# wheretrue/exon

Hardware: AMD Instinct MI355X
Metric: Mrows/sec filter+agg on 1B-row synthetic VCF; achieved HBM GB/s vs peak (higher is better)
Workload: dtype f64

## Files before the change

### exon_amd/_lib.py

```python
import ctypes as C
import os
import subprocess

_HERE = os.path.dirname(os.path.abspath(__file__))
LIB_PATH = os.environ.get("EXON_HIP_LIB") or os.path.join(_HERE, "lib", "libexon_hip.so")
CSRC = os.path.join(_HERE, "csrc")


class ExonHipError(RuntimeError):
    def __init__(self, code, msg):
        super().__init__(f"exon_hip status {code}: {msg}")
        self.code = code


class ArrowSchema(C.Structure):
    pass


ArrowSchema._fields_ = [
    ("format", C.c_char_p), ("name", C.c_char_p), ("metadata", C.c_char_p), ("flags", C.c_int64),
    ("n_children", C.c_int64), ("children", C.POINTER(C.POINTER(ArrowSchema))),
    ("dictionary", C.POINTER(ArrowSchema)), ("release", C.c_void_p), ("private_data", C.c_void_p),
]

# ... 39 lines not shown
        ("lmax", C.c_int32), ("y_type", C.c_int32),
        ("columns", C.c_int32 * 4),
    ]


class BgzfBlock(C.Structure):
    _fields_ = [("comp_offset", C.c_uint32), ("comp_size", C.c_uint32), ("out_offset", C.c_uint32), ("out_size", C.c_uint32),
                ("crc32", C.c_uint32), ("reserved", C.c_uint32)]


class BAMColumns(C.Structure):
    _fields_ = [("n_rows", C.c_int64), ("n_undecided", C.c_int64), ("consumed_bytes", C.c_int64), ("flag", C.c_void_p),
                ("mapq", C.c_void_p), ("mapq_valid", C.c_void_p), ("ref_id", C.c_void_p), ("ref_valid", C.c_void_p),
                ("start", C.c_void_p), ("end", C.c_void_p), ("pos_valid", C.c_void_p)]


class FASTQViews(C.Structure):
    _fields_ = [("n_reads", C.c_int64), ("n_undecided", C.c_int64), ("consumed_bytes", C.c_int64),
                ("seq_start", C.c_void_p), ("seq_end", C.c_void_p), ("qual_start", C.c_void_p), ("qual_end", C.c_void_p),
                ("text_base", C.c_void_p), ("head_start", C.c_void_p), ("head_end", C.c_void_p)]


class FASTAViews(C.Structure):
    _fields_ = [("n_records", C.c_int64), ("n_undecided", C.c_int64), ("consumed_bytes", C.c_int64), ("n_lines", C.c_int64),
                ("seq_bytes", C.c_int64), ("text_base", C.c_void_p), ("text_bytes", C.c_int64), ("first_line_start", C.c_int64),
                ("head_start", C.c_void_p), ("head_end", C.c_void_p), ("seq_offsets", C.c_void_p), ("line_end", C.c_void_p),
                ("line_dst", C.c_void_p)]


class VCFColumns(C.Structure):
    _fields_ = [("n_rows", C.c_int64), ("n_undecided", C.c_int64), ("chrom_id", C.c_void_p), ("pos", C.c_void_p),
                ("pos_valid", C.c_void_p), ("qual", C.c_void_p), ("qual_valid", C.c_void_p), ("filter_id", C.c_void_p),
                ("info", C.c_void_p), ("info_valid", C.c_void_p), ("consumed_bytes", C.c_int64),
                ("n_info", C.c_int32), ("reserved", C.c_int32), ("infos", C.c_void_p * 16), ("infos_valid", C.c_void_p * 16),
                ("info_kinds", C.c_char * 16), ("list_offsets", C.c_void_p * 16), ("list_item_valid", C.c_void_p * 16),
                ("info_nulls", C.c_int32 * 16)]


class GFFColumns(C.Structure):
    _fields_ = [("n_rows", C.c_int64), ("n_undecided", C.c_int64), ("consumed_bytes", C.c_int64),
                ("seqname_id", C.c_void_p), ("source_id", C.c_void_p), ("type_id", C.c_void_p), ("start", C.c_void_p),
                ("end", C.c_void_p), ("score", C.c_void_p), ("score_valid", C.c_void_p), ("strand_id", C.c_void_p),
                ("strand_valid", C.c_void_p), ("phase_id", C.c_void_p), ("phase_valid", C.c_void_p)]


class GFFAttributes(C.Structure):
    _fields_ = [("n_entries", C.c_int64), ("n_items", C.c_int64), ("n_key_bytes", C.c_int64), ("n_item_bytes", C.c_int64),
                ("n_undecided", C.c_int64), ("map_offsets", C.c_void_p), ("key_offsets", C.c_void_p), ("key_values", C.c_void_p),
                ("list_offsets", C.c_void_p), ("item_offsets", C.c_void_p), ("item_values", C.c_void_p)]


class VCFInfoText(C.Structure):
    _fields_ = [("n_bytes", C.c_int64), ("n_undecided", C.c_int64), ("offsets", C.c_void_p), ("values", C.c_void_p)]


class GTFAttributes(C.Structure):
    _fields_ = [("n_entries", C.c_int64), ("n_key_bytes", C.c_int64), ("n_value_bytes", C.c_int64), ("n_undecided", C.c_int64),
                ("map_offsets", C.c_void_p), ("key_offsets", C.c_void_p), ("key_values", C.c_void_p),
                ("value_offsets", C.c_void_p), ("value_values", C.c_void_p)]


class BEDColumns(C.Structure):
    _fields_ = [("n_rows", C.c_int64), ("n_undecided", C.c_int64), ("consumed_bytes", C.c_int64),
                ("chrom_id", C.c_void_p), ("start", C.c_void_p), ("end", C.c_void_p), ("score", C.c_void_p), ("score_valid", C.c_void_p),
                ("strand_id", C.c_void_p), ("strand_valid", C.c_void_p), ("name_off", C.c_void_p), ("name_len", C.c_void_p),
                ("name_valid", C.c_void_p), ("text", C.c_void_p)]


class ScanOptions(C.Structure):
    _fields_ = [("format", C.c_int32), ("compression", C.c_int32), ("batch_size", C.c_int64),
                ("info_field", C.c_char_p), ("region", C.c_char_p), ("use_index", C.c_int32), ("gpu_parse", C.c_int32),
                ("projection", C.c_uint64)]


class GzipStats(C.Structure):
    _fields_ = [(n, C.c_uint64) for n in ("calls", "chunks", "repairs", "overflow_retries", "members", "comp_bytes", "out_bytes")]


FORMATS = {"vcf": 1, "bam": 2, "fastq": 3, "fasta": 4, "sam": 5, "bcf": 6, "cram": 7, "gff": 8, "gtf": 9, "bed": 10}
COMPRESSION = {"auto": 0, None: 0, "none": 1, "gzip": 2}
PROJECT_VCF_FORMATS_ON_DEVICE = 32
PROJECT_BED = {"name": 1 << 3, "score": 1 << 4, "strand": 1 << 5, "thick_start": 1 << 6, "thick_end": 1 << 7, "color": 1 << 8,
               "block_count": 1 << 9, "block_sizes": 1 << 10, "block_starts": 1 << 11}

PLAN_REGION_COUNT = 2
PLAN_FLAG_MAPQ_GROUP_COUNT = 3
PLAN_CMP_AVG_BY_GROUP = 4
PLAN_QUAL_POS_HIST = 5
PLAN_OVERLAP_COUNT = 6
PLAN_WITHIN_COUNT = 7
PLAN_CMP_MINMAX_BY_GROUP = 8
PLAN_READ_STATS_HIST = 9
PLAN_SEQ_STATS_HIST = 10
LAUNCH_ACCUMULATE = 0
LAUNCH_OVERWRITE = 1
CMP = {">": 0, ">=": 1, "<": 2, "<=": 3, "=": 4, "==": 4, "!=": 5, "<>": 5}
REGION_OPEN_END = 2**63 - 1

_vp, _i32, _i64, _u64, _dbl = C.c_void_p, C.c_int32, C.c_int64, C.c_uint64, C.c_double
_colp = C.POINTER(Column)

ALLGATHER_FN = C.CFUNCTYPE(C.c_int, C.c_void_p, C.c_void_p, C.c_void_p, C.c_size_t)

SIGNATURES = {
    "exon_hip_abi_version": (C.c_int, []),
    "exon_hip_device_count": (C.c_int, [C.POINTER(C.c_int)]),
    "exon_hip_ctx_create": (C.c_int, [C.c_int, C.POINTER(_vp)]),
    "exon_hip_ctx_destroy": (C.c_int, [_vp]),
    "exon_hip_ctx_info": (C.c_int, [_vp, C.POINTER(DeviceInfo)]),
    "exon_hip_last_error": (C.c_char_p, [_vp]),
    "exon_hip_malloc": (C.c_int, [_vp, C.c_size_t, C.POINTER(_vp)]),
    "exon_hip_free": (C.c_int, [_vp, _vp]),
    "exon_hip_memcpy_h2d": (C.c_int, [_vp, _vp, _vp, C.c_size_t, _vp]),
    "exon_hip_memcpy_d2h": (C.c_int, [_vp, _vp, _vp, C.c_size_t, _vp]),
    "exon_hip_memset": (C.c_int, [_vp, _vp, C.c_int, C.c_size_t, _vp]),
    "exon_hip_sync": (C.c_int, [_vp, _vp]),
    "exon_hip_read_probe": (C.c_int, [_vp, _vp, C.POINTER(_vp), _i32, _i64, _i32, C.POINTER(_dbl), C.POINTER(_i64)]),
    "exon_hip_timer_start": (C.c_int, [_vp, _vp]),
    "exon_hip_timer_stop_ms": (C.c_int, [_vp, _vp, C.POINTER(C.c_float)]),
    "exon_hip_region_count": (C.c_int, [_vp, _vp, _colp, _colp, _i64, _i32, _i64, _i64, _vp]),
    "exon_hip_overlap_count": (C.c_int, [_vp, _vp, _colp, _colp, _colp, _i64, _i32, _i64, _i64, _vp]),
    "exon_hip_within_count": (C.c_int, [_vp, _vp, _colp, _colp, _colp, _i64, _i32, _i64, _i64, _vp]),
    "exon_hip_flag_mapq_group_count": (C.c_int, [_vp, _vp, _colp, _colp, _colp, _i64, _i32, _i32, _i32, _i32, _vp]),
    "exon_hip_cmp_avg_by_group": (C.c_int, [_vp, _vp, _colp, _colp, _colp, _i64, _dbl, _i32, _i32, _vp, _vp]),
    "exon_hip_cmp_minmax_by_group": (C.c_int, [_vp, _vp, _colp, _colp, _colp, _i64, _dbl, _i32, _i32, _vp]),
    "exon_hip_minmax_decode": (C.c_int, [_vp, _i64, _i32, _i32, _vp, _vp]),
    "exon_hip_qual_pos_hist": (C.c_int, [_vp, _vp, _colp, _i64, _i32, _vp]),
    "exon_hip_gen_c6": (C.c_int, [_vp, _vp, _u64, _i64, _i64, _vp, _vp, _vp, _vp, _vp]),
    "exon_hip_gen_c2": (C.c_int, [_vp, _vp, _u64, _i64, _i64, _i64, _vp, _vp]),
    "exon_hip_gen_c3": (C.c_int, [_vp, _vp, _u64, _i64, _i64, _vp, _vp, _vp, _vp, _vp]),
    "exon_hip_gen_c4": (C.c_int, [_vp, _vp, _u64, _i64, _i64, _vp, _vp, _vp, _vp, _vp]),
    "exon_hip_gen_c5": (C.c_int, [_vp, _vp, _u64, _i64, _i64, _i32, _vp, _vp]),
    "exon_hip_parse_region": (C.c_int, [C.c_char_p, C.c_char_p, C.c_size_t, C.POINTER(_i64), C.POINTER(_i64)]),
    "exon_hip_regroup_files_by_size": (C.c_int, [C.POINTER(_i64), _i32, _i32, C.POINTER(_i32)]),
    "exon_hip_plan_create": (C.c_int, [_vp, C.POINTER(PlanDesc), C.POINTER(_vp)]),
    "exon_hip_plan_destroy": (C.c_int, [_vp]),
    "exon_hip_plan_state_size": (C.c_int, [_vp, C.POINTER(_i64), C.POINTER(_i64)]),
    "exon_hip_plan_launch": (C.c_int, [_vp, _vp, _colp, _i32, _i64, _i32, _vp]),
    "exon_hip_plan_launch_chunks": (C.c_int, [_vp, _vp, _colp, _i32, _i32, _vp, _i32, _vp]),
    "exon_hip_fold_states": (C.c_int, [_vp, _vp, _vp, _i32, _i64, _i64, _vp]),
    "exon_hip_merge_states": (C.c_int, [_vp, _vp, _vp, _vp, _i64, _i64, _vp, _vp]),
    "exon_hip_plan_fold_states": (C.c_int, [_vp, _vp, _vp, _i32, _vp]),
    "exon_hip_rccl_unique_id": (C.c_int, [_vp]),
    "exon_hip_rccl_comm_init": (C.c_int, [_vp, _vp, _i32, _i32, C.POINTER(_vp)]),
    "exon_hip_rccl_comm_destroy": (C.c_int, [_vp]),
    "exon_hip_comm_wrap_rccl": (C.c_int, [_vp, C.POINTER(_vp)]),
    "exon_hip_comm_from_callbacks": (C.c_int, [_i32, _i32, ALLGATHER_FN, _vp, C.POINTER(_vp)]),
    "exon_hip_rccl_comm_count": (C.c_int, [_vp, C.POINTER(_i32), C.POINTER(_i32)]),
    "exon_hip_stream_reset": (C.c_int, [_vp]),
    "exon_hip_stream_open": (C.c_int, [_vp, _i32, C.POINTER(_vp)]),
    "exon_hip_stream_push": (C.c_int, [_vp, C.POINTER(ArrowArray)]),
    "exon_hip_stream_push_device": (C.c_int, [_vp, C.POINTER(ArrowDeviceArray)]),
    "exon_hip_stream_state": (C.c_int, [_vp, C.POINTER(_vp), C.POINTER(_vp), C.POINTER(_vp)]),
    "exon_hip_stream_all_reduce": (C.c_int, [_vp, _vp]),
    "exon_hip_stream_keys": (C.c_int, [_vp, _vp, C.c_size_t, C.POINTER(_i32), C.POINTER(C.c_size_t), C.POINTER(_i32)]),
    "exon_hip_stream_set_keys": (C.c_int, [_vp, C.c_char_p, C.c_size_t, _i32]),
    "exon_hip_keys_union": (C.c_int, [C.c_char_p, C.c_size_t, C.POINTER(_i32), _i32, _vp, C.c_size_t, C.POINTER(_i32),
                                      C.POINTER(C.c_size_t), C.POINTER(_i32)]),
    "exon_hip_stream_reconcile_keys": (C.c_int, [_vp, _vp]),
    "exon_hip_stream_set_region_contig": (C.c_int, [_vp, C.c_char_p]),
    "exon_hip_stream_sync": (C.c_int, [_vp]),
    "exon_hip_stream_finish": (C.c_int, [_vp, _vp, _vp]),
    "exon_hip_stream_finish_arrow": (C.c_int, [_vp, C.POINTER(ArrowArray), C.POINTER(ArrowSchema)]),
    "exon_hip_stream_close": (C.c_int, [_vp]),
    "exon_hip_scan_open": (C.c_int, [C.c_char_p, C.POINTER(ScanOptions), C.POINTER(_vp)]),
    "exon_hip_scan_schema": (C.c_int, [_vp, C.POINTER(ArrowSchema)]),
# ... 101 lines not shown
```

### exon_amd/csrc/gpu_parse.hip

```cpp
#include <hip/hip_runtime.h>

#include <cstring>
#include <string>
#include <vector>

#include "host/decimal_f32.h"
#include "internal.h"
#include "list_kernels.h"

namespace {

constexpr int TPB = 256;
constexpr int FILTER_SLOTS = 8192;
constexpr int FILTER_POOL = EXON_DICT_POOL;

__host__ __device__ inline uint64_t fnv1a(const uint8_t* p, int n) {
  uint64_t h = 0xCBF29CE484222325ULL;
  for (int i = 0; i < n; ++i) {
    h ^= p[i];
    h *= 0x100000001B3ULL;
  }
  return h | 1ULL;
}

// ... 175 lines not shown
  }
  int read_back(exon_hip_ctx* ctx, hipStream_t s) {
    HIP_TRY(ctx, hipGetLastError());
    HIP_TRY(ctx, hipMemcpyAsync(h_scalars, d_scalars, 16, hipMemcpyDeviceToHost, s));
    HIP_TRY(ctx, hipStreamSynchronize(s));
    return EXON_HIP_OK;
  }
  int64_t consumed(unsigned skip) const { return h_scalars[2] > skip ? (int64_t)h_scalars[2] - skip : 0; }
};

__global__ void k_last_newline(const unsigned* __restrict__ nl_pos, unsigned* __restrict__ scalars, unsigned cap) {
  const unsigned n = scalars[0];
  scalars[2] = (n && n <= cap) ? nl_pos[n - 1] + 1u : 0u;
}

struct NameTable {
  const uint64_t* keys;
  const int32_t* ids;
  const uint32_t* text_off;
  const uint32_t* text_len;
  const uint8_t* pool;
  int mask;
};

struct FilterTable {
  unsigned long long* keys;
  int32_t* ids;
  uint32_t* text_off;
  uint32_t* text_len;
  uint8_t* pool;
  int32_t* counters;
};

constexpr int MAX_INFO = EXON_HIP_MAX_INFO_FIELDS;
struct InfoKeys {
  int n;
  int len[MAX_INFO];
  int off[MAX_INFO];
  char kind[MAX_INFO];
  const uint8_t* text;
};
struct ParseOut {
  int32_t* chrom_id;
  int64_t* pos;
  uint8_t* pos_valid;
  float* qual;
  uint8_t* qual_valid;
  int32_t* filter_id;
  uint32_t* filter_off;
  uint32_t* filter_len;
  float* info[MAX_INFO];
  uint8_t* info_valid[MAX_INFO];
  uint32_t* lv_off[MAX_INFO];
  uint32_t* lv_cnt[MAX_INFO];
  unsigned* exceptions;
};

__device__ __forceinline__ void store_valid(uint8_t* bm, int64_t row0_of_wave, int64_t n_rows, bool v, int lane) {
  const unsigned long long m = __ballot(v);
  if (lane < 8) {
    const int64_t r = row0_of_wave + lane * 8;
    if (r < n_rows) bm[r >> 3] = (uint8_t)(m >> (lane * 8));
  }
}

__device__ __forceinline__ unsigned eq_mask16(const uint4& v, uint32_t splat) {
  const uint32_t w[4] = {v.x, v.y, v.z, v.w};
  unsigned mask = 0;
#pragma unroll
  for (int k = 0; k < 4; ++k) {
    const uint32_t x = w[k] ^ splat;
    const uint32_t m = ~(((x & 0x7F7F7F7Fu) + 0x7F7F7F7Fu) | x | 0x7F7F7F7Fu);
    const uint32_t t = m >> 7;
    mask |= ((t | (t >> 7) | (t >> 14) | (t >> 21)) & 0xFu) << (4 * k);
  }
  return mask;
}
__device__ __forceinline__ unsigned clip_mask16(unsigned mask, unsigned a, unsigned begin, unsigned end) {
  if (begin > a) mask &= 0xFFFFu << (begin - a);
  if (end - a < 16u) mask &= (1u << (end - a)) - 1u;
  return mask;
}

__global__ __launch_bounds__(TPB) void k_parse_lines(const uint8_t* __restrict__ text, const unsigned* __restrict__ nl_pos,
                                                     const unsigned* __restrict__ n_lines_p, NameTable contigs,
                                                     FilterTable filters, InfoKeys ik, ParseOut out, unsigned cap, unsigned skip,
                                                     unsigned n_total) {
  const int64_t n_rows = min(*n_lines_p, cap);
  auto group16 = [&](unsigned a) {
    uint4 v = {0, 0, 0, 0};
    if (a + 16u <= n_total) {
      v = *reinterpret_cast<const uint4*>(text + a);
    } else {
      unsigned* w = &v.x;
      for (unsigned i = 0; a + i < n_total; ++i) w[i >> 2] |= (unsigned)text[a + i] << (8 * (i & 3));
    }
    return v;
  };
  const int64_t row = (int64_t)blockIdx.x * TPB + threadIdx.x;
  const int lane = threadIdx.x & 63;
  bool pos_ok = false, qual_ok = false, bad = false;
  unsigned info_ok = 0;
  if (row < n_rows) {
    const unsigned begin = row ? nl_pos[row - 1] + 1 : skip;
    unsigned end = nl_pos[row];
    if (end > begin && text[end - 1] == '\r') --end;
    unsigned fs[9];
    int nf = 0;
    fs[0] = begin;
    for (unsigned a = begin & ~15u; a < end && nf < 8; a += 16) {
      unsigned m = clip_mask16(eq_mask16(group16(a), 0x09090909u), a, begin, end);
      while (m && nf < 8) {
        fs[++nf] = a + (unsigned)__ffs((int)m);
        m &= m - 1;
      }
    }
    auto fbeg = [&](int f) { return fs[f]; };
    auto fend = [&](int f) { return f < nf ? fs[f + 1] - 1 : end; };
    if (nf < 7 || begin == end || text[begin] == '#') {
      bad = true;
      out.chrom_id[row] = 0;
      out.pos[row] = 0;
      out.qual[row] = 0.f;
      out.filter_id[row] = -1;
      for (int q = 0; q < ik.n; ++q)
        if (ik.kind[q] == 'F' || ik.kind[q] == 'I') out.lv_cnt[q][row] = 0;
    } else {
#ifndef EXON_PARSE_SKIP
#define EXON_PARSE_SKIP 0
#endif
      if (!(EXON_PARSE_SKIP & 1)) {
        const uint8_t* p = text + fbeg(0);
        const int len = (int)(fend(0) - fbeg(0));
        const uint64_t h = fnv1a(p, len);
        int slot = (int)(h & (uint64_t)contigs.mask), id = -1;
        for (int probe = 0; probe <= contigs.mask; ++probe) {
          const uint64_t k = contigs.keys[slot];
          if (k == 0) break;
          if (k == h && (int)contigs.text_len[slot] == len) {
            bool same = true;
            for (int i = 0; i < len && same; ++i) same = contigs.pool[contigs.text_off[slot] + i] == p[i];
            if (same) {
              id = contigs.ids[slot];
              break;
            }
          }
          slot = (slot + 1) & contigs.mask;
        }
        if (id < 0) bad = true;
        out.chrom_id[row] = id < 0 ? 0 : id;
      }
      if (!(EXON_PARSE_SKIP & 2)) {
        uint64_t v = 0;
        unsigned pb = fbeg(1), pn = fend(1) - fbeg(1);
        if (pn && text[pb] == '+') ++pb, --pn;
        bool ok = pn > 0;
        if (pn <= 16 && pb + 16u <= n_total) {
          uint64_t w[2];
          __builtin_memcpy(w, text + pb, 16);
          for (unsigned k = 0; k < pn; ++k) {
            const unsigned d = ((unsigned)(w[k >> 3] >> (8 * (k & 7))) & 0xFFu) - (unsigned)'0';
            ok &= d <= 9u;
            v = v * 10 + d;
          }
        } else {
          for (unsigned i = pb; i < pb + pn && ok; ++i) {
            const uint8_t c = text[i];
            if (c < '0' || c > '9') ok = false;
            else v = v * 10 + (c - '0');
          }
        }
        if (pn > 18) ok = false;
        pos_ok = ok && v > 0;
        if (!ok) bad = true;
        out.pos[row] = pos_ok ? (int64_t)v : 0;
      }
      if (!(EXON_PARSE_SKIP & 4)) {
        const int len = (int)(fend(5) - fbeg(5));
        float q = 0.f;
        if (!(len == 1 && text[fbeg(5)] == '.')) {
          uint32_t bits;
          if (exon::dec::parse_f32(reinterpret_cast<const char*>(text + fbeg(5)), len, &bits)) {
            q = __uint_as_float(bits);
            qual_ok = true;
          } else {
            bad = true;
          }
        }
        out.qual[row] = q;
      }
      if (!(EXON_PARSE_SKIP & 8)) {
        const uint8_t* p = text + fbeg(6);
        int len = (int)(fend(6) - fbeg(6));
        if (len == 1 && p[0] == '.') len = 0;
        const unsigned long long h = fnv1a(p, len);
        int slot = (int)(h & (FILTER_SLOTS - 1));
        int found = -1;
        for (int probe = 0; probe < FILTER_SLOTS; ++probe) {
          unsigned long long k = filters.keys[slot];
          if (k == 0) {
            k = atomicCAS(&filters.keys[slot], 0ull, h);
            if (k == 0) {
              filters.text_off[slot] = fbeg(6);
              filters.text_len[slot] = (uint32_t)len;
              found = slot;
              break;
            }
          }
          if (k == h) {
            found = slot;
            break;
          }
          slot = (slot + 1) & (FILTER_SLOTS - 1);
        }
        if (found < 0) atomicExch(&filters.counters[2], 1);
        out.filter_id[row] = found;
        out.filter_off[row] = fbeg(6);
        out.filter_len[row] = (uint32_t)len;
      }
      if (ik.n > 0 && !(EXON_PARSE_SKIP & 16)) {
        unsigned seen = 0;
        int left = ik.n;
        const unsigned ib = fbeg(7), ie = fend(7);
        if (!(ie - ib == 1 && text[ib] == '.')) {
          unsigned i = ib;
          auto entry = [&](unsigned j) {
            for (int q = 0; q < ik.n; ++q) {
              const int kl = ik.len[q];
              if ((seen >> q & 1u) || (int)(j - i) < kl) continue;
              const bool valued = (int)(j - i) > kl && text[i + kl] == '=';
              if (!valued && (int)(j - i) != kl) continue;
              bool same = true;
              for (int k = 0; k < kl && same; ++k) same = text[i + k] == ik.text[ik.off[q] + k];
              if (!same) continue;
              seen |= 1u << q;
              --left;
              if (ik.kind[q] == 'b') {
                info_ok |= 1u << q;
              } else if (valued) {
                const unsigned vb = i + kl + 1;
                const int vl = (int)(j - vb);
                if (!(vl == 0 || (vl == 1 && text[vb] == '.'))) {
                  uint32_t bits;
                  if (ik.kind[q] == 's') {
                    out.lv_off[q][row] = vb;
                    out.lv_cnt[q][row] = (uint32_t)vl;
                    info_ok |= 1u << q;
                  } else if (ik.kind[q] == 'F' || ik.kind[q] == 'I') {
                    unsigned items = 1;
                    for (int k = 0; k < vl; ++k) items += text[vb + k] == ',';
                    out.lv_off[q][row] = vb;
                    out.lv_cnt[q][row] = items;
                    info_ok |= 1u << q;
                  } else if (ik.kind[q] == 'i') {
                    int k = 0;
                    const bool neg = text[vb] == '-';
                    if (neg || text[vb] == '+') k = 1;
                    int64_t iv = 0;
                    bool ok = k < vl && vl - k <= 10;
                    for (; k < vl && ok; ++k) {
                      const unsigned d = (unsigned)text[vb + k] - '0';
                      ok = d <= 9u;
                      iv = iv * 10 + d;
                    }
                    if (neg) iv = -iv;
                    if (ok && iv >= INT32_MIN && iv <= INT32_MAX) {
                      out.info[q][row] = __int_as_float((int32_t)iv);
                      info_ok |= 1u << q;
                    } else {
                      bad = true;
                    }
                  } else if (exon::dec::parse_f32(reinterpret_cast<const char*>(text + vb), vl, &bits)) {
                    out.info[q][row] = __uint_as_float(bits);
                    info_ok |= 1u << q;
                  } else {
                    bad = true;
                  }
                }
              }
            }
            i = j + 1;
          };
          for (unsigned a = ib & ~15u; a < ie && left > 0; a += 16) {
            unsigned m = clip_mask16(eq_mask16(group16(a), 0x3B3B3B3Bu), a, ib, ie);
            while (m && left > 0) {
              entry(a + (unsigned)__ffs((int)m) - 1u);
              m &= m - 1;
            }
          }
          if (left > 0 && i < ie) entry(ie);
        }
        for (int q = 0; q < ik.n; ++q) {
          if (info_ok >> q & 1u) continue;
          if (ik.kind[q] == 'F' || ik.kind[q] == 'I') out.lv_cnt[q][row] = 0;
          else if (ik.kind[q] != 'b') out.info[q][row] = 0.f;
        }
      }
    }
  }
  const int64_t wave_row0 = row - lane;
  store_valid(out.pos_valid, wave_row0, n_rows, pos_ok, lane);
  store_valid(out.qual_valid, wave_row0, n_rows, qual_ok, lane);
  for (int q = 0; q < ik.n; ++q) store_valid(out.info_valid[q], wave_row0, n_rows, (info_ok >> q & 1u) != 0, lane);
  const unsigned long long nb = __ballot(bad);
  if (lane == 0 && nb) atomicAdd(out.exceptions, (unsigned)__popcll(nb));
}

__global__ __launch_bounds__(TPB) void k_info_string_ids(const uint8_t* __restrict__ text, const uint32_t* __restrict__ voff, const uint32_t* __restrict__ vlen,
                                                         const uint8_t* __restrict__ valid, const unsigned* __restrict__ n_lines_p, unsigned cap, FilterTable t,
                                                         int32_t* __restrict__ ids, int null_as_value) {
  const unsigned n = min(*n_lines_p, cap);
  const unsigned row = blockIdx.x * TPB + threadIdx.x;
  bool has = false;
  if (row < n) {
    has = (valid[row >> 3] >> (row & 7)) & 1;
    int found = -1;
    if (has || null_as_value) {
      const uint8_t* p = text + (has ? voff[row] : 0u);
      const int len = has ? (int)vlen[row] : 0;
      const unsigned long long h = fnv1a(p, len);
      int slot = (int)(h & (FILTER_SLOTS - 1));
      found = -1;
      for (int probe = 0; probe < FILTER_SLOTS; ++probe) {
        unsigned long long k = t.keys[slot];
        if (k == 0) {
          k = atomicCAS(&t.keys[slot], 0ull, h);
          if (k == 0) {
            t.text_off[slot] = has ? voff[row] : 0u;
            t.text_len[slot] = (uint32_t)len;
            found = slot;
            break;
          }
        }
        if (k == h) {
          found = slot;
          break;
        }
        slot = (slot + 1) & (FILTER_SLOTS - 1);
      }
      if (found < 0) atomicExch(&t.counters[2], 1);
    }
    ids[row] = found;
  }
  const unsigned long long miss = __ballot(row < n && !has && !null_as_value);
  if ((threadIdx.x & 63) == 0 && miss) atomicAdd(&t.counters[3], __popcll(miss));
}

__global__ __launch_bounds__(256) void k_assign_filters(const uint8_t* __restrict__ text, FilterTable f) {
  for (int s = threadIdx.x; s < FILTER_SLOTS; s += 256)
    if (f.keys[s] != 0 && f.ids[s] == -1) {
      const uint32_t len = f.text_len[s], src = f.text_off[s];
      const int id = atomicAdd(&f.counters[0], 1);
      const int po = atomicAdd(&f.counters[1], (int)len);
      if (id >= EXON_HIP_MAX_GROUPS || po < 0 || po + (int64_t)len > FILTER_POOL) {
        f.counters[2] = 1;
        f.ids[s] = -2;
        continue;
      }
      for (uint32_t i = 0; i < len; ++i) f.pool[po + i] = text[src + i];
      f.text_off[s] = (uint32_t)po;
      f.ids[s] = id;
    }
}

__global__ __launch_bounds__(TPB) void k_remap_filters(int32_t* __restrict__ ids_io, const unsigned* __restrict__ n_lines_p, unsigned cap,
                                                       FilterTable t, const uint8_t* __restrict__ text, const uint32_t* __restrict__ off,
                                                       const uint32_t* __restrict__ len, const uint8_t* __restrict__ valid) {
  const int64_t n = min(*n_lines_p, cap);
  const bool check = t.counters[2] == 0;
  bool differs = false;
  for (int64_t i = (int64_t)blockIdx.x * TPB + threadIdx.x; i < n; i += (int64_t)gridDim.x * TPB) {
    const unsigned slot = (unsigned)ids_io[i];
    if (slot >= (unsigned)FILTER_SLOTS) {
      ids_io[i] = 0;
      continue;
    }
    const int id = t.ids[slot];
    ids_io[i] = id < 0 ? 0 : id;
    if (!check) continue;
    const bool has = !valid || ((valid[i >> 3] >> (i & 7)) & 1);
    const uint32_t l = has ? len[i] : 0u, to = t.text_off[slot];
    if (t.text_len[slot] != l || (uint64_t)to + l > (uint64_t)FILTER_POOL) {
      differs = true;
      continue;
    }
    const uint8_t* a = text + (has ? off[i] : 0u);
    const uint8_t* b = t.pool + to;
// ... 1569 lines not shown
```

### exon_amd/csrc/host/decimal_f32.h

```cpp
#pragma once
#include <stdint.h>

#if defined(__HIPCC__)
#include <hip/hip_runtime.h>
#define EXON_HD __host__ __device__ __forceinline__
#else
#define EXON_HD inline
#endif

namespace exon {
namespace dec {

constexpr int kSmallestPow10 = -65, kLargestPow10 = 38;

#if defined(__HIP_DEVICE_COMPILE__)
__device__
#endif
static const uint64_t kPow5[104][2] = {
    {0x86ccbb52ea94baeaULL, 0x98e947129fc2b4e9ULL},
    {0xa87fea27a539e9a5ULL, 0x3f2398d747b36224ULL},
    {0xd29fe4b18e88640eULL, 0x8eec7f0d19a03aadULL},
    {0x83a3eeeef9153e89ULL, 0x1953cf68300424acULL},
    {0xa48ceaaab75a8e2bULL, 0x5fa8c3423c052dd7ULL},
    {0xcdb02555653131b6ULL, 0x3792f412cb06794dULL},
// ... 75 lines not shown
    {0x8e1bc9bf04000000ULL, 0x0000000000000000ULL},
    {0xb1a2bc2ec5000000ULL, 0x0000000000000000ULL},
    {0xde0b6b3a76400000ULL, 0x0000000000000000ULL},
    {0x8ac7230489e80000ULL, 0x0000000000000000ULL},
    {0xad78ebc5ac620000ULL, 0x0000000000000000ULL},
    {0xd8d726b7177a8000ULL, 0x0000000000000000ULL},
    {0x878678326eac9000ULL, 0x0000000000000000ULL},
    {0xa968163f0a57b400ULL, 0x0000000000000000ULL},
    {0xd3c21bcecceda100ULL, 0x0000000000000000ULL},
    {0x84595161401484a0ULL, 0x0000000000000000ULL},
    {0xa56fa5b99019a5c8ULL, 0x0000000000000000ULL},
    {0xcecb8f27f4200f3aULL, 0x0000000000000000ULL},
    {0x813f3978f8940984ULL, 0x4000000000000000ULL},
    {0xa18f07d736b90be5ULL, 0x5000000000000000ULL},
    {0xc9f2c9cd04674edeULL, 0xa400000000000000ULL},
    {0xfc6f7c4045812296ULL, 0x4d00000000000000ULL},
    {0x9dc5ada82b70b59dULL, 0xf020000000000000ULL},
    {0xc5371912364ce305ULL, 0x6c28000000000000ULL},
    {0xf684df56c3e01bc6ULL, 0xc732000000000000ULL},
    {0x9a130b963a6c115cULL, 0x3c7f400000000000ULL},
    {0xc097ce7bc90715b3ULL, 0x4b9f100000000000ULL},
    {0xf0bdc21abb48db20ULL, 0x1e86d40000000000ULL},
    {0x96769950b50d88f4ULL, 0x1314448000000000ULL},
};

EXON_HD void mul64(uint64_t a, uint64_t b, uint64_t* hi, uint64_t* lo) {
#if defined(__HIP_DEVICE_COMPILE__)
  *lo = a * b;
  *hi = __umul64hi(a, b);
#else
  const unsigned __int128 p = (unsigned __int128)a * b;
  *lo = (uint64_t)p;
  *hi = (uint64_t)(p >> 64);
#endif
}
EXON_HD int clz64(uint64_t x) {
#if defined(__HIP_DEVICE_COMPILE__)
  return __clzll((long long)x);
#else
  return __builtin_clzll(x);
#endif
}

EXON_HD uint32_t eisel_lemire_f32(uint64_t w, int q) {
  if (q < kSmallestPow10) return 0u;
  if (q > kLargestPow10) return 0x7F800000u;
  const int lz = clz64(w);
  w <<= lz;
  uint64_t hi, lo;
  mul64(w, kPow5[q - kSmallestPow10][0], &hi, &lo);
  const uint64_t precision_mask = 0xFFFFFFFFFFFFFFFFULL >> 26;
  if ((hi & precision_mask) == precision_mask) {
    uint64_t hi2, lo2;
    mul64(w, kPow5[q - kSmallestPow10][1], &hi2, &lo2);
    lo += hi2;
    if (hi2 > lo) ++hi;
  }
  const int upperbit = (int)(hi >> 63);
  const int shift = upperbit + 64 - 23 - 3;
  uint64_t mantissa = hi >> shift;
  int power2 = (int)((((152170 + 65536) * (int64_t)q) >> 16) + 63) + upperbit - lz + 127;
  if (power2 <= 0) {
    if (-power2 + 1 >= 64) return 0u;
    mantissa >>= -power2 + 1;
    mantissa += (mantissa & 1);
    mantissa >>= 1;
    power2 = (mantissa < (1ULL << 23)) ? 0 : 1;
    return ((uint32_t)power2 << 23) | (uint32_t)(mantissa & 0x7FFFFF);
  }
  if (lo <= 1 && q >= -17 && q <= 10 && (mantissa & 3) == 1) {
    if ((mantissa << shift) == hi) mantissa &= ~1ULL;
  }
  mantissa += (mantissa & 1);
  mantissa >>= 1;
  if (mantissa >= (2ULL << 23)) {
    mantissa = 1ULL << 23;
    ++power2;
  }
  mantissa &= ~(1ULL << 23);
  if (power2 >= 0xFF) return 0x7F800000u;
  return ((uint32_t)power2 << 23) | (uint32_t)mantissa;
}

EXON_HD int parse_f32(const char* p, int n, uint32_t* bits) {
  int i = 0;
  uint32_t sign = 0;
  if (i < n && (p[i] == '-' || p[i] == '+')) sign = (p[i++] == '-') ? 0x80000000u : 0u;
  uint64_t w = 0;
  unsigned nz = 0;
  int digits = 0, q = 0;
  const int i0 = i;
  for (; i < n; ++i) {
    const unsigned d = (unsigned)(unsigned char)p[i] - (unsigned)'0';
    if (d > 9u) break;
    w = w * 10 + d;
    nz |= d;
    digits += nz != 0;
  }
  int nd = i - i0;
  if (i < n && p[i] == '.') {
    const int f0 = ++i;
    for (; i < n; ++i) {
      const unsigned d = (unsigned)(unsigned char)p[i] - (unsigned)'0';
      if (d > 9u) break;
      w = w * 10 + d;
      nz |= d;
      digits += nz != 0;
    }
    q = f0 - i;
    nd += i - f0;
  }
  if (nd == 0) return 0;
  if (digits > 19) return 0;
  if (i < n && (p[i] == 'e' || p[i] == 'E')) {
    ++i;
    bool eneg = false;
    if (i < n && (p[i] == '-' || p[i] == '+')) eneg = p[i++] == '-';
    int e = 0, ed = 0;
    for (; i < n && p[i] >= '0' && p[i] <= '9'; ++i, ++ed)
      if (e < 100000) e = e * 10 + (p[i] - '0');
    if (ed == 0) return 0;
    q += eneg ? -e : e;
  }
  if (i != n) return 0;
  if (w == 0) {
    *bits = sign;
    return 1;
  }
  if (w < (1ull << 24) && q <= 0 && q >= -10) {
    const float p10[11] = {1.f, 10.f, 100.f, 1e3f, 1e4f, 1e5f, 1e6f, 1e7f, 1e8f, 1e9f, 1e10f};
    const float r = (float)(uint32_t)w / p10[-q];
    uint32_t rb;
    __builtin_memcpy(&rb, &r, 4);
    *bits = sign | rb;
    return 1;
  }
  *bits = sign | eisel_lemire_f32(w, q < -100000 ? -100000 : (q > 100000 ? 100000 : q));
  return 1;
}

}
}
```

Baseline: 553,400.

## Stage each wavefront's line text in LDS before parsing VCF fields

The parse kernel now has each 64-row wavefront cooperatively copy its contiguous span of text into shared memory with coalesced 16-byte loads when the span fits a fixed budget. Per-row field scanning, hashing and number parsing then read from LDS through a templated source abstraction, falling back to global memory when the span is too large. The goal is to replace scattered, uncoalesced per-thread byte reads of global memory with one coalesced load per wave. The filter-table insert is also changed to serialize same-slot CAS attempts within a wave through a leader lane. In exchange, each block uses about 22 KB of LDS, which may lower occupancy, and the leader loop adds some control overhead.

```diff
diff --git a/exon_amd/_lib.py b/exon_amd/_lib.py
--- a/exon_amd/_lib.py
+++ b/exon_amd/_lib.py
@@ -145,6 +145,7 @@
 PROJECT_VCF_FORMATS_ON_DEVICE = 32
 PROJECT_BED = {"name": 1 << 3, "score": 1 << 4, "strand": 1 << 5, "thick_start": 1 << 6, "thick_end": 1 << 7, "color": 1 << 8,
                "block_count": 1 << 9, "block_sizes": 1 << 10, "block_starts": 1 << 11}
+PARSE_WAVE_TEXT_BYTES = 5632
 
 PLAN_REGION_COUNT = 2
 PLAN_FLAG_MAPQ_GROUP_COUNT = 3
diff --git a/exon_amd/csrc/gpu_parse.hip b/exon_amd/csrc/gpu_parse.hip
--- a/exon_amd/csrc/gpu_parse.hip
+++ b/exon_amd/csrc/gpu_parse.hip
@@ -281,34 +281,77 @@
   return mask;
 }
 
-__global__ __launch_bounds__(TPB) void k_parse_lines(const uint8_t* __restrict__ text, const unsigned* __restrict__ nl_pos,
-                                                     const unsigned* __restrict__ n_lines_p, NameTable contigs,
-                                                     FilterTable filters, InfoKeys ik, ParseOut out, unsigned cap, unsigned skip,
-                                                     unsigned n_total) {
-  const int64_t n_rows = min(*n_lines_p, cap);
-  auto group16 = [&](unsigned a) {
+#ifndef EXON_PARSE_WAVE_TEXT
+#define EXON_PARSE_WAVE_TEXT 5632
+#endif
+constexpr unsigned PARSE_WAVE_TEXT = EXON_PARSE_WAVE_TEXT;
+static_assert(PARSE_WAVE_TEXT % 16 == 0, "whole 16-byte groups");
+constexpr unsigned PARSE_WAVE_GROUPS = PARSE_WAVE_TEXT / 16 + 3;
+
+struct GlobalText {
+  const uint8_t* __restrict__ text;
+  unsigned n_total;
+  __device__ __forceinline__ unsigned byte(unsigned o) const { return text[o]; }
+  __device__ __forceinline__ uint4 group16(unsigned a) const {
     uint4 v = {0, 0, 0, 0};
     if (a + 16u <= n_total) {
       v = *reinterpret_cast<const uint4*>(text + a);
     } else {
-      unsigned* w = &v.x;
-      for (unsigned i = 0; a + i < n_total; ++i) w[i >> 2] |= (unsigned)text[a + i] << (8 * (i & 3));
+      unsigned w[4] = {0, 0, 0, 0};
+#pragma unroll
+      for (unsigned i = 0; i < 16; ++i)
+        if (a + i < n_total) w[i >> 2] |= (unsigned)text[a + i] << (8 * (i & 3));
+      v = make_uint4(w[0], w[1], w[2], w[3]);
     }
     return v;
-  };
-  const int64_t row = (int64_t)blockIdx.x * TPB + threadIdx.x;
-  const int lane = threadIdx.x & 63;
+  }
+  __device__ __forceinline__ bool load16(unsigned o, uint64_t& w0, uint64_t& w1) const {
+    if (o + 16u > n_total) return false;
+    __builtin_memcpy(&w0, text + o, 8);
+    __builtin_memcpy(&w1, text + o + 8, 8);
+    return true;
+  }
+};
+struct LdsText {
+  const uint8_t* s;
+  unsigned base;
+  __device__ __forceinline__ unsigned byte(unsigned o) const { return s[o - base]; }
+  __device__ __forceinline__ uint4 group16(unsigned a) const { return *reinterpret_cast<const uint4*>(s + (a - base)); }
+  __device__ __forceinline__ bool load16(unsigned o, uint64_t& w0, uint64_t& w1) const {
+    const unsigned r = o - base, sh = (r & 7u) * 8u;
+    const uint64_t* p = reinterpret_cast<const uint64_t*>(s + (r & ~7u));
+    const uint64_t x0 = p[0], x1 = p[1], x2 = p[2];
+    w0 = sh ? (x0 >> sh) | (x1 << (64u - sh)) : x0;
+    w1 = sh ? (x1 >> sh) | (x2 << (64u - sh)) : x1;
+    return true;
+  }
+};
+
+template <class Src>
+__device__ __forceinline__ uint64_t fnv1a_text(const Src& src, unsigned off, int n) {
+  uint64_t h = 0xCBF29CE484222325ULL;
+  for (int i = 0; i < n; ++i) h = (h ^ (uint64_t)src.byte(off + (unsigned)i)) * 0x100000001B3ULL;
+  return h | 1ULL;
+}
+
+struct RowFlags {
   bool pos_ok = false, qual_ok = false, bad = false;
   unsigned info_ok = 0;
-  if (row < n_rows) {
-    const unsigned begin = row ? nl_pos[row - 1] + 1 : skip;
-    unsigned end = nl_pos[row];
-    if (end > begin && text[end - 1] == '\r') --end;
+};
+
+template <class Src>
+__device__ __forceinline__ void parse_line(const Src& src, int64_t row, unsigned begin, unsigned end, const NameTable& contigs,
+                                           const FilterTable& filters, const InfoKeys& ik, const ParseOut& out, RowFlags& fl) {
+  bool &pos_ok = fl.pos_ok, &qual_ok = fl.qual_ok, &bad = fl.bad;
+  unsigned& info_ok = fl.info_ok;
+  const int lane = threadIdx.x & 63;
+  {
+    if (end > begin && src.byte(end - 1) == '\r') --end;
     unsigned fs[9];
     int nf = 0;
     fs[0] = begin;
     for (unsigned a = begin & ~15u; a < end && nf < 8; a += 16) {
-      unsigned m = clip_mask16(eq_mask16(group16(a), 0x09090909u), a, begin, end);
+      unsigned m = clip_mask16(eq_mask16(src.group16(a), 0x09090909u), a, begin, end);
       while (m && nf < 8) {
         fs[++nf] = a + (unsigned)__ffs((int)m);
         m &= m - 1;
@@ -316,7 +359,7 @@
     }
     auto fbeg = [&](int f) { return fs[f]; };
     auto fend = [&](int f) { return f < nf ? fs[f + 1] - 1 : end; };
-    if (nf < 7 || begin == end || text[begin] == '#') {
+    if (nf < 7 || begin == end || src.byte(begin) == '#') {
       bad = true;
       out.chrom_id[row] = 0;
       out.pos[row] = 0;
@@ -329,16 +372,17 @@
 #define EXON_PARSE_SKIP 0
 #endif
       if (!(EXON_PARSE_SKIP & 1)) {
-        const uint8_t* p = text + fbeg(0);
-        const int len = (int)(fend(0) - fbeg(0));
-        const uint64_t h = fnv1a(p, len);
+        const unsigned cb = fbeg(0);
+        const int len = (int)(fend(0) - cb);
+        const uint64_t h = fnv1a_text(src, cb, len);
         int slot = (int)(h & (uint64_t)contigs.mask), id = -1;
         for (int probe = 0; probe <= contigs.mask; ++probe) {
           const uint64_t k = contigs.keys[slot];
           if (k == 0) break;
           if (k == h && (int)contigs.text_len[slot] == len) {
+            const uint32_t po = contigs.text_off[slot];
             bool same = true;
-            for (int i = 0; i < len && same; ++i) same = contigs.pool[contigs.text_off[slot] + i] == p[i];
+            for (int i = 0; i < len && same; ++i) same = contigs.pool[po + i] == src.byte(cb + (unsigned)i);
             if (same) {
               id = contigs.ids[slot];
               break;
@@ -352,21 +396,21 @@
       if (!(EXON_PARSE_SKIP & 2)) {
         uint64_t v = 0;
         unsigned pb = fbeg(1), pn = fend(1) - fbeg(1);
-        if (pn && text[pb] == '+') ++pb, --pn;
+        if (pn && src.byte(pb) == '+') ++pb, --pn;
         bool ok = pn > 0;
-        if (pn <= 16 && pb + 16u <= n_total) {
-          uint64_t w[2];
-          __builtin_memcpy(w, text + pb, 16);
-          for (unsigned k = 0; k < pn; ++k) {
-            const unsigned d = ((unsigned)(w[k >> 3] >> (8 * (k & 7))) & 0xFFu) - (unsigned)'0';
-            ok &= d <= 9u;
+        uint64_t w0 = 0, w1 = 0;
+        const bool fast = src.load16(pb, w0, w1) && pn <= 16;
+        const unsigned pnf = fast ? pn : 0u;
+        for (unsigned k = 0; k < pnf; ++k) {
+          const unsigned d = ((unsigned)((k < 8 ? w0 : w1) >> (8 * (k & 7))) & 0xFFu) - (unsigned)'0';
+          ok &= d <= 9u;
+          v = v * 10 + d;
+        }
+        if (!fast) {
+          for (unsigned k = 0; k < pn && ok; ++k) {
+            const unsigned d = src.byte(pb + k) - (unsigned)'0';
+            ok = d <= 9u;
             v = v * 10 + d;
-          }
-        } else {
-          for (unsigned i = pb; i < pb + pn && ok; ++i) {
-            const uint8_t c = text[i];
-            if (c < '0' || c > '9') ok = false;
-            else v = v * 10 + (c - '0');
           }
         }
         if (pn > 18) ok = false;
@@ -375,11 +419,12 @@
         out.pos[row] = pos_ok ? (int64_t)v : 0;
       }
       if (!(EXON_PARSE_SKIP & 4)) {
-        const int len = (int)(fend(5) - fbeg(5));
+        const unsigned qb = fbeg(5);
+        const int len = (int)(fend(5) - qb);
         float q = 0.f;
-        if (!(len == 1 && text[fbeg(5)] == '.')) {
+        if (!(len == 1 && src.byte(qb) == '.')) {
           uint32_t bits;
-          if (exon::dec::parse_f32(reinterpret_cast<const char*>(text + fbeg(5)), len, &bits)) {
+          if (exon::dec::parse_f32_at([&](int i) { return (unsigned char)src.byte(qb + (unsigned)i); }, len, &bits)) {
             q = __uint_as_float(bits);
             qual_ok = true;
           } else {
@@ -389,18 +434,30 @@
         out.qual[row] = q;
       }
       if (!(EXON_PARSE_SKIP & 8)) {
-        const uint8_t* p = text + fbeg(6);
-        int len = (int)(fend(6) - fbeg(6));
-        if (len == 1 && p[0] == '.') len = 0;
-        const unsigned long long h = fnv1a(p, len);
+        const unsigned fb = fbeg(6);
+        int len = (int)(fend(6) - fb);
+        if (len == 1 && src.byte(fb) == '.') len = 0;
+        const unsigned long long h = fnv1a_text(src, fb, len);
         int slot = (int)(h & (FILTER_SLOTS - 1));
         int found = -1;
         for (int probe = 0; probe < FILTER_SLOTS; ++probe) {
           unsigned long long k = filters.keys[slot];
           if (k == 0) {
-            k = atomicCAS(&filters.keys[slot], 0ull, h);
+            bool pending = true;
+            while (pending) {
+              const int leader = __ffsll((long long)__ballot(true)) - 1;
+              const unsigned long long lh = __shfl(h, leader);
+              const int ls = __shfl(slot, leader);
+              if (lh == h && ls == slot) {
+                unsigned long long r = 0;
+                if (lane == leader) r = atomicCAS(&filters.keys[slot], 0ull, h);
+                r = __shfl(r, leader);
+                k = (lane == leader || r != 0) ? r : h;
+                pending = false;
+              }
+            }
             if (k == 0) {
-              filters.text_off[slot] = fbeg(6);
+              filters.text_off[slot] = fb;
               filters.text_len[slot] = (uint32_t)len;
               found = slot;
               break;
@@ -414,23 +471,24 @@
         }
         if (found < 0) atomicExch(&filters.counters[2], 1);
         out.filter_id[row] = found;
-        out.filter_off[row] = fbeg(6);
+        out.filter_off[row] = fb;
         out.filter_len[row] = (uint32_t)len;
       }
       if (ik.n > 0 && !(EXON_PARSE_SKIP & 16)) {
         unsigned seen = 0;
         int left = ik.n;
         const unsigned ib = fbeg(7), ie = fend(7);
-        if (!(ie - ib == 1 && text[ib] == '.')) {
+        if (!(ie - ib == 1 && src.byte(ib) == '.')) {
           unsigned i = ib;
           auto entry = [&](unsigned j) {
+            const int el = (int)(j - i);
             for (int q = 0; q < ik.n; ++q) {
               const int kl = ik.len[q];
-              if ((seen >> q & 1u) || (int)(j - i) < kl) continue;
-              const bool valued = (int)(j - i) > kl && text[i + kl] == '=';
-              if (!valued && (int)(j - i) != kl) continue;
+              if ((seen >> q & 1u) || el < kl) continue;
+              const bool valued = el > kl && src.byte(i + (unsigned)kl) == '=';
+              if (!valued && el != kl) continue;
               bool same = true;
-              for (int k = 0; k < kl && same; ++k) same = text[i + k] == ik.text[ik.off[q] + k];
+              for (int k = 0; k < kl && same; ++k) same = src.byte(i + (unsigned)k) == ik.text[ik.off[q] + k];
               if (!same) continue;
               seen |= 1u << q;
               --left;
@@ -439,7 +497,7 @@
               } else if (valued) {
                 const unsigned vb = i + kl + 1;
                 const int vl = (int)(j - vb);
-                if (!(vl == 0 || (vl == 1 && text[vb] == '.'))) {
+                if (!(vl == 0 || (vl == 1 && src.byte(vb) == '.'))) {
                   uint32_t bits;
                   if (ik.kind[q] == 's') {
                     out.lv_off[q][row] = vb;
@@ -447,18 +505,18 @@
                     info_ok |= 1u << q;
                   } else if (ik.kind[q] == 'F' || ik.kind[q] == 'I') {
                     unsigned items = 1;
-                    for (int k = 0; k < vl; ++k) items += text[vb + k] == ',';
+                    for (int k = 0; k < vl; ++k) items += src.byte(vb + (unsigned)k) == ',';
                     out.lv_off[q][row] = vb;
                     out.lv_cnt[q][row] = items;
                     info_ok |= 1u << q;
                   } else if (ik.kind[q] == 'i') {
-                    int k = 0;
-                    const bool neg = text[vb] == '-';
-                    if (neg || text[vb] == '+') k = 1;
+                    const unsigned c0 = src.byte(vb);
+                    const bool neg = c0 == '-';
+                    int k = (neg || c0 == '+') ? 1 : 0;
                     int64_t iv = 0;
                     bool ok = k < vl && vl - k <= 10;
                     for (; k < vl && ok; ++k) {
-                      const unsigned d = (unsigned)text[vb + k] - '0';
+                      const unsigned d = src.byte(vb + (unsigned)k) - '0';
                       ok = d <= 9u;
                       iv = iv * 10 + d;
                     }
@@ -469,7 +527,7 @@
                     } else {
                       bad = true;
                     }
-                  } else if (exon::dec::parse_f32(reinterpret_cast<const char*>(text + vb), vl, &bits)) {
+                  } else if (exon::dec::parse_f32_at([&](int x) { return (unsigned char)src.byte(vb + (unsigned)x); }, vl, &bits)) {
                     out.info[q][row] = __uint_as_float(bits);
                     info_ok |= 1u << q;
                   } else {
@@ -481,7 +539,7 @@
             i = j + 1;
           };
           for (unsigned a = ib & ~15u; a < ie && left > 0; a += 16) {
-            unsigned m = clip_mask16(eq_mask16(group16(a), 0x3B3B3B3Bu), a, ib, ie);
+            unsigned m = clip_mask16(eq_mask16(src.group16(a), 0x3B3B3B3Bu), a, ib, ie);
             while (m && left > 0) {
               entry(a + (unsigned)__ffs((int)m) - 1u);
               m &= m - 1;
@@ -497,11 +555,47 @@
       }
     }
   }
-  const int64_t wave_row0 = row - lane;
-  store_valid(out.pos_valid, wave_row0, n_rows, pos_ok, lane);
-  store_valid(out.qual_valid, wave_row0, n_rows, qual_ok, lane);
-  for (int q = 0; q < ik.n; ++q) store_valid(out.info_valid[q], wave_row0, n_rows, (info_ok >> q & 1u) != 0, lane);
-  const unsigned long long nb = __ballot(bad);
+}
+
+__global__ __launch_bounds__(TPB) void k_parse_lines(const uint8_t* __restrict__ text, const unsigned* __restrict__ nl_pos,
+                                                     const unsigned* __restrict__ n_lines_p, NameTable contigs,
+                                                     FilterTable filters, InfoKeys ik, ParseOut out, unsigned cap, unsigned skip,
+                                                     unsigned n_total) {
+  __shared__ uint4 s_text[TPB / 64][PARSE_WAVE_GROUPS];
+  const int64_t n_rows = min(*n_lines_p, cap);
+  const GlobalText slab{text, n_total};
+  const int lane = threadIdx.x & 63;
+  const int wave = __builtin_amdgcn_readfirstlane((int)(threadIdx.x >> 6));
+  const int64_t wave_row0 = (int64_t)blockIdx.x * TPB + wave * 64;
+  const int64_t row = wave_row0 + lane;
+  RowFlags fl;
+  if (wave_row0 < n_rows) {
+    const int64_t last = min(wave_row0 + 63, n_rows - 1);
+    const unsigned span_b = wave_row0 ? nl_pos[wave_row0 - 1] + 1 : skip;
+    const unsigned span_e = nl_pos[last];
+    const bool staged = span_e + 1u - span_b <= PARSE_WAVE_TEXT;
+    unsigned begin = 0, end = 0;
+    if (row < n_rows) {
+      begin = row ? nl_pos[row - 1] + 1 : skip;
+      end = nl_pos[row];
+    }
+    if (staged) {
+      uint4* s = s_text[wave];
+      const unsigned base = span_b & ~15u;
+      const unsigned groups = (span_e - base + 15u) >> 4;
+      for (unsigned g = lane; g < groups; g += 64) s[g] = slab.group16(base + 16u * g);
+      __builtin_amdgcn_fence(__ATOMIC_RELEASE, "wavefront");
+      __builtin_amdgcn_wave_barrier();
+      __builtin_amdgcn_fence(__ATOMIC_ACQUIRE, "wavefront");
+      if (row < n_rows) parse_line(LdsText{reinterpret_cast<const uint8_t*>(s), base}, row, begin, end, contigs, filters, ik, out, fl);
+    } else {
+      if (row < n_rows) parse_line(slab, row, begin, end, contigs, filters, ik, out, fl);
+    }
+  }
+  store_valid(out.pos_valid, wave_row0, n_rows, fl.pos_ok, lane);
+  store_valid(out.qual_valid, wave_row0, n_rows, fl.qual_ok, lane);
+  for (int q = 0; q < ik.n; ++q) store_valid(out.info_valid[q], wave_row0, n_rows, (fl.info_ok >> q & 1u) != 0, lane);
+  const unsigned long long nb = __ballot(fl.bad);
   if (lane == 0 && nb) atomicAdd(out.exceptions, (unsigned)__popcll(nb));
 }
 
diff --git a/exon_amd/csrc/host/decimal_f32.h b/exon_amd/csrc/host/decimal_f32.h
--- a/exon_amd/csrc/host/decimal_f32.h
+++ b/exon_amd/csrc/host/decimal_f32.h
@@ -181,26 +181,30 @@
   return ((uint32_t)power2 << 23) | (uint32_t)mantissa;
 }
 
-EXON_HD int parse_f32(const char* p, int n, uint32_t* bits) {
+template <class At>
+EXON_HD int parse_f32_at(At at, int n, uint32_t* bits) {
   int i = 0;
   uint32_t sign = 0;
-  if (i < n && (p[i] == '-' || p[i] == '+')) sign = (p[i++] == '-') ? 0x80000000u : 0u;
+  if (n > 0) {
+    const unsigned char c0 = at(0);
+    if (c0 == '-' || c0 == '+') sign = (c0 == '-') ? 0x80000000u : 0u, i = 1;
+  }
   uint64_t w = 0;
   unsigned nz = 0;
   int digits = 0, q = 0;
   const int i0 = i;
   for (; i < n; ++i) {
-    const unsigned d = (unsigned)(unsigned char)p[i] - (unsigned)'0';
+    const unsigned d = (unsigned)(unsigned char)at(i) - (unsigned)'0';
     if (d > 9u) break;
     w = w * 10 + d;
     nz |= d;
     digits += nz != 0;
   }
   int nd = i - i0;
-  if (i < n && p[i] == '.') {
+  if (i < n && at(i) == '.') {
     const int f0 = ++i;
     for (; i < n; ++i) {
-      const unsigned d = (unsigned)(unsigned char)p[i] - (unsigned)'0';
+      const unsigned d = (unsigned)(unsigned char)at(i) - (unsigned)'0';
       if (d > 9u) break;
       w = w * 10 + d;
       nz |= d;
@@ -211,13 +215,13 @@
   }
   if (nd == 0) return 0;
   if (digits > 19) return 0;
-  if (i < n && (p[i] == 'e' || p[i] == 'E')) {
+  if (i < n && (at(i) == 'e' || at(i) == 'E')) {
     ++i;
     bool eneg = false;
-    if (i < n && (p[i] == '-' || p[i] == '+')) eneg = p[i++] == '-';
+    if (i < n && (at(i) == '-' || at(i) == '+')) eneg = at(i++) == '-';
     int e = 0, ed = 0;
-    for (; i < n && p[i] >= '0' && p[i] <= '9'; ++i, ++ed)
-      if (e < 100000) e = e * 10 + (p[i] - '0');
+    for (; i < n && at(i) >= '0' && at(i) <= '9'; ++i, ++ed)
+      if (e < 100000) e = e * 10 + (at(i) - '0');
     if (ed == 0) return 0;
     q += eneg ? -e : e;
   }
@@ -238,5 +242,9 @@
   return 1;
 }
 
-}
-}
+EXON_HD int parse_f32(const char* p, int n, uint32_t* bits) {
+  return parse_f32_at([p](int i) { return (unsigned char)p[i]; }, n, bits);
+}
+
+}
+}
```

Result: no change. 549,200 (-0.8%).
